# ctxnn/GenConViT

Hardware: AMD Instinct MI355X
Metric: frames/sec (224x224, ed+vae forward) (higher is better)
Workload: dtype f16

## Files before the change

genconvit_amd/_lib.py:

```python
from __future__ import annotations

import ctypes
import ctypes.util
import json
import os
import threading

_HERE = os.path.dirname(os.path.abspath(__file__))
LIB_PATH = os.environ.get("GCV_LIB_PATH") or os.path.join(_HERE, "lib", "libgenconvit_hip.so")

GCV_F32, GCV_BF16, GCV_F16 = 0, 1, 2
ACT_NONE, ACT_RELU, ACT_GELU, ACT_LEAKY = 0, 1, 2, 3
A_PLAIN, A_IM2COL3_POOL, A_IM2COL3_S2 = 0, 1, 2
EPI_BIAS_ACT, EPI_RESID, EPI_POOL4, EPI_CONVT, EPI_SPLITK = 0, 1, 2, 3, 4

c_void_p, c_int, c_int64, c_float, c_char_p, c_size_t = (ctypes.c_void_p, ctypes.c_int, ctypes.c_int64,
                                                         ctypes.c_float, ctypes.c_char_p, ctypes.c_size_t)


class TensorDesc(ctypes.Structure):
    _fields_ = [("name", c_char_p), ("data", c_void_p), ("numel", c_int64), ("on_device", c_int)]


class GemmArgs(ctypes.Structure):
# ... 30 lines not shown
    "gcv_comm_unique_id": (c_int, [c_void_p]),
    "gcv_comm_create": (c_int, [ctypes.POINTER(c_void_p), c_int, c_int, c_void_p, c_int]),
    "gcv_comm_destroy": (None, [c_void_p]),
    "gcv_allgather_logits": (c_int, [c_void_p, c_void_p, c_int, c_void_p, c_void_p]),
    "gcv_convnext_forward": (c_int, [c_void_p, c_int, c_void_p, c_int, c_int, c_void_p, c_void_p]),
    "gcv_swin_forward": (c_int, [c_void_p, c_void_p, c_int, c_void_p, c_void_p]),
    "gcv_vote": (c_int, [c_void_p, c_int, c_void_p, c_void_p]),
    "gcv_preprocess": (c_int, [c_int, c_void_p, c_void_p, c_int, c_int, c_int, c_void_p]),
    "gcv_face_crop_resize": (c_int, [c_void_p, c_int, c_int, c_int, c_void_p, c_int, c_void_p, c_int, c_void_p]),
    "gcv_cam_overlay": (c_int, [c_void_p, c_int, c_int, c_int, c_void_p, c_int, c_void_p, c_int, c_int, c_void_p, c_float,
                                c_int, c_void_p, c_void_p]),
    "gcv_vote_segments": (c_int, [c_void_p, c_int, c_int, c_void_p, c_int, c_void_p, c_void_p]),
    "gcv_tap_set": (c_int, [c_void_p, c_char_p, c_void_p, c_size_t]),
    "gcv_tap_clear": (c_int, [c_void_p]),
    "gcv_tap_written": (c_int, [c_void_p, c_char_p]),
    "gcv_profile_enable": (c_int, [c_void_p, c_int]),
    "gcv_profile_report": (c_char_p, [c_void_p]),
    "gcv_k_gemm": (c_int, [c_int, c_int, c_int, ctypes.POINTER(GemmArgs), c_void_p]),
    "gcv_k_stem_ln": (c_int, [c_int, c_void_p, c_int64, c_int64, c_int64, c_int64, c_void_p, c_void_p, c_void_p,
                              c_void_p, c_void_p, c_int, c_int, c_int, c_float, c_void_p]),
    "gcv_k_stem_ln_c": (c_int, [c_int, c_void_p, c_int64, c_int64, c_int64, c_int64, c_void_p, c_void_p, c_void_p,
                                c_void_p, c_void_p, c_int, c_int, c_int, c_int, c_float, c_void_p]),
    "gcv_k_dwconv7_ln": (c_int, [c_int, c_void_p, c_void_p, c_void_p, c_void_p, c_void_p, c_void_p, c_int, c_int,
                                 c_int, c_int, c_float, c_void_p]),
    "gcv_dw_plan": (c_int, [c_int, c_int, c_int, c_int, c_int, c_int, c_void_p]),
    "gcv_convnext_res_ok": (c_int, [c_int, c_int]),
    "gcv_k_ln_patchify": (c_int, [c_int, c_void_p, c_void_p, c_void_p, c_void_p, c_int, c_int, c_int, c_int, c_float,
                                  c_void_p]),
    "gcv_k_layernorm_rows": (c_int, [c_int, c_void_p, c_void_p, c_void_p, c_void_p, c_int64, c_int, c_float, c_void_p]),
    "gcv_k_pool_ln": (c_int, [c_int, c_void_p, c_void_p, c_void_p, c_void_p, c_int, c_int, c_int, c_float, c_void_p]),
    "gcv_k_conv3_first": (c_int, [c_int, c_void_p, c_int64, c_int64, c_int64, c_int64, c_void_p, c_void_p, c_void_p,
                                  c_int, c_int, c_int, c_int, c_int, c_void_p]),
    "gcv_k_convt2_small": (c_int, [c_int, c_void_p, c_void_p, c_void_p, c_void_p, c_int, c_int, c_int, c_int, c_void_p]),
    "gcv_k_reparam": (c_int, [c_int, c_void_p, c_int, c_void_p, c_void_p, c_void_p, c_void_p, c_int, c_int, c_void_p]),
    "gcv_k_head_tail": (c_int, [c_int, c_void_p, c_void_p, c_void_p, c_void_p, c_int, c_int, c_void_p]),
    "gcv_k_head_tail_splitk": (c_int, [c_int, c_void_p, c_int, c_void_p, c_int, c_void_p, c_void_p, c_void_p, c_int, c_int,
                                       c_void_p]),
    "gcv_k_resize_mse": (c_int, [c_int, c_void_p, c_void_p, c_void_p, c_void_p, c_void_p, c_int, c_void_p]),
    "gcv_k_swin_window_attn": (c_int, [c_int, c_void_p, c_void_p, c_void_p, c_int, c_int, c_int, c_int, c_int, c_int,
                                       c_void_p]),
    "gcv_k_patch_merge_ln": (c_int, [c_int, c_void_p, c_void_p, c_void_p, c_void_p, c_int, c_int, c_int, c_int, c_float,
                                     c_void_p]),
    "gcv_k_mean_tokens": (c_int, [c_int, c_void_p, c_void_p, c_int, c_int, c_int, c_void_p]),
    "gcv_k_fused_mlp": (c_int, [c_int, c_int, c_void_p, c_void_p, c_void_p, c_void_p, c_void_p, c_void_p, c_void_p,
                                c_void_p, c_int, c_void_p]),
    "gcv_k_fused_mlp_lnp": (c_int, [c_int, c_int, c_void_p, c_void_p, c_void_p, c_void_p, c_void_p, c_void_p, c_void_p,
                                    c_void_p, c_void_p, c_float, c_int, c_void_p, c_void_p, c_void_p, c_void_p, c_void_p,
                                    c_int, c_void_p]),
    "gcv_k_fused_mlp_timed": (c_int, [c_int, c_int, c_void_p, c_void_p, c_void_p, c_void_p, c_void_p, c_void_p,
                                      c_void_p, c_void_p, c_int, c_int, c_void_p, c_void_p]),
}

_lib = None
_lock = threading.Lock()


class GenConViTHipError(RuntimeError):
    pass


def _preload_hip_runtime():
    cands = []
    try:
        import torch
        cands.append(os.path.join(os.path.dirname(torch.__file__), "lib", "libamdhip64.so"))
    except Exception:
# ... 483 lines not shown
```

genconvit_amd/csrc/api.hip:

```cpp
#include "../../include/genconvit_hip.h"

#include <dlfcn.h>

#include <cstdio>
#include <cstdlib>
#include <cstring>
#include <map>
#include <mutex>
#include <set>
#include <sstream>
#include <vector>

#include "cnx_mlp.h"
#include "gemm.h"
#include "kernels.h"
#include "net.h"

namespace gcv {
static thread_local std::string g_err;
void set_error(const std::string& msg) { g_err = msg; }
const char* get_error() { return g_err.c_str(); }

int ensure_dynamic_lds(const void* fn, int bytes) {
  static std::mutex mu;
  static std::map<std::pair<const void*, int>, int> done;
  int dev = 0;
  GCV_CHECK_HIP(hipGetDevice(&dev));
  std::lock_guard<std::mutex> lk(mu);
  auto it = done.find({fn, dev});
  if (it != done.end() && it->second >= bytes) return 0;
  GCV_CHECK_HIP(hipFuncSetAttribute(fn, hipFuncAttributeMaxDynamicSharedMemorySize, bytes));
  done[{fn, dev}] = bytes;
  return 0;
}

hipEvent_t Profiler::get_event() {
  if (next_event == pool.size()) {
    hipEvent_t e;
    if (hipEventCreate(&e) != hipSuccess) return nullptr;
    pool.push_back(e);
  }
  return pool[next_event++];
}
Profiler::~Profiler() {
  for (hipEvent_t e : pool) (void)hipEventDestroy(e);
}
// ... 574 lines not shown
    return rc;
  };
  DISPATCH_DT(dtype, put(dw_plan<T>(p, nimg, H, W, C, aligned != 0)));
}

int gcv_convnext_res_ok(int arch, int res) { return cnx_res_ok(arch, res) ? 1 : 0; }

int gcv_k_ln_patchify(int dtype, const void* x, const float* w, const float* b, void* out, int nimg, int H, int W,
                      int C, float eps, gcv_stream s) {
  DISPATCH_DT(dtype, launch_ln_patchify<T>((const T*)x, w, b, (T*)out, nimg, H, W, C, eps, (hipStream_t)s));
}

int gcv_k_layernorm_rows(int dtype, const void* x, const float* w, const float* b, void* out, int64_t rows, int C,
                         float eps, gcv_stream s) {
  DISPATCH_DT(dtype, launch_layernorm_rows<T>((const T*)x, w, b, (T*)out, rows, C, eps, (hipStream_t)s));
}

int gcv_k_pool_ln(int dtype, const void* x, const float* w, const float* b, void* out, int nimg, int HW, int C,
                  float eps, gcv_stream s) {
  DISPATCH_DT(dtype, launch_pool_ln<T>((const T*)x, w, b, (T*)out, nimg, HW, C, eps, (hipStream_t)s));
}

int gcv_k_conv3_first(int dtype, const void* x, int64_t sb, int64_t sc, int64_t sy, int64_t sx, const float* wp,
                      const float* bias, void* out, int nimg, int H, int W, int pool, int act, gcv_stream s) {
  DISPATCH_DT(dtype, launch_conv3_first<T>((const T*)x, sb, sc, sy, sx, wp, bias, (T*)out, nimg, H, W, pool != 0, act,
                                           (hipStream_t)s));
}

int gcv_k_convt2_small(int dtype, const void* x, const float* wp, const float* bias, void* out, int nimg, int H,
                       int W, int act, gcv_stream s) {
  DISPATCH_DT(dtype, launch_convt2_small<T>((const T*)x, wp, bias, (T*)out, nimg, H, W, act, (hipStream_t)s));
}

int gcv_k_reparam(int dtype, const float* partial, int splitk, const float* bias, const float* eps, float* mu_out,
                  void* z_nhwc, int B, int N, gcv_stream s) {
  DISPATCH_DT(dtype, launch_reparam<T>(partial, splitk, bias, eps, mu_out, (T*)z_nhwc, B, N, (hipStream_t)s));
}

int gcv_k_head_tail(int dtype, const void* h, const float* w, const float* bias, float* logits, int B, int K,
                    gcv_stream s) {
  DISPATCH_DT(dtype, launch_head_tail<T>((const T*)h, w, bias, logits, B, K, (hipStream_t)s));
}

int gcv_k_head_tail_splitk(int dtype, const float* partial, int splitk, const float* b1, int act, const float* w,
                           const float* bias, float* logits, int B, int K, gcv_stream s) {
  DISPATCH_DT(dtype, launch_head_tail_splitk<T>(partial, splitk, b1, act, w, bias, logits, B, K, (hipStream_t)s));
}

int gcv_k_resize_mse(int dtype, const void* xhat, const void* img, void* recon, float* msepart, float* mse, int B,
                     gcv_stream s) {
  DISPATCH_DT(dtype, launch_resize_mse<T>((const T*)xhat, (const T*)img, (T*)recon, msepart, mse, B, (hipStream_t)s));
}

int gcv_k_swin_window_attn(int dtype, const void* qkv, const float* rpb, void* out, int nimg, int H, int W, int C,
                           int nH, int shift, gcv_stream s) {
  DISPATCH_DT(dtype, launch_swin_window_attn<T>((const T*)qkv, rpb, (T*)out, nimg, H, W, C, nH, shift, (hipStream_t)s));
}

int gcv_k_patch_merge_ln(int dtype, const void* x, const float* w, const float* b, void* out, int nimg, int H, int W,
                         int C, float eps, gcv_stream s) {
  DISPATCH_DT(dtype, launch_patch_merge_ln<T>((const T*)x, w, b, (T*)out, nimg, H, W, C, eps, (hipStream_t)s));
}

int gcv_k_mean_tokens(int dtype, const void* x, void* out, int nimg, int L, int C, gcv_stream s) {
  DISPATCH_DT(dtype, launch_mean_tokens<T>((const T*)x, (T*)out, nimg, L, C, (hipStream_t)s));
}
// ... 51 lines not shown
```

genconvit_amd/csrc/net_impl.h:

```cpp
#pragma once
#include <algorithm>
#include <cmath>
#include <cstdlib>
#include <cstring>

#include "cam.h"
#include "cam_bwd.h"
#include "cnx_mlp.h"
#include "gemm.h"
#include "kernels.h"
#include "net.h"
#include "swin.h"

namespace gcv {

template <typename T> inline T host_cvt(float v);
template <> inline float host_cvt<float>(float v) { return v; }
template <> inline half_t host_cvt<half_t>(float v) { return (half_t)v; }
template <> inline bf16_t host_cvt<bf16_t>(float v) {
  uint32_t u;
  std::memcpy(&u, &v, 4);
  uint16_t h;
  if ((u & 0x7fffffffu) > 0x7f800000u) h = (uint16_t)((u >> 16) | 0x40);
  else h = (uint16_t)((u + 0x7fffu + ((u >> 16) & 1u)) >> 16);
  bf16_t r;
  std::memcpy(&r, &h, 2);
  return r;
}

struct WeightStore {
  std::vector<void*> ptrs;
  size_t bytes = 0;
  ~WeightStore() { clear(); }
  void clear() {
    for (void* p : ptrs) (void)hipFree(p);
    ptrs.clear();
    bytes = 0;
  }
  void* raw(size_t n) {
    void* p = nullptr;
    if (hipMalloc(&p, n ? n : 16) != hipSuccess) return nullptr;
// ... 803 lines not shown
                       Dw + (int64_t)tok0[p] * C3, B, side3[p], 1e-6f};
        GCV_TRY(run("explain2.dw_ln_bwd", 2.0 * 49 * B * hw3[p] * C3, (sizeof(T) + 8.0) * (double)B * hw3[p] * C3,
                    [&] { return launch_dw_ln_bwd<T>(da, C3, cur); }));
        GCV_TRY(run("explain2.dw_dgrad_res", 2.0 * 49 * B * hw3[p] * C3, 12.0 * (double)B * hw3[p] * C3, [&] {
          return launch_dw_dgrad_res(Dw + (int64_t)tok0[p] * C3, k.dw_w, G + (int64_t)tok0[p] * C3, B, side3[p], C3, cur);
        }));
      }
    }
    GCV_TRY(run("explain2.scale_rows", 2.0 * M * C3, (sizeof(T) + 4.0) * (double)M * C3,
                [&] { return launch_scale_rows<T>(G, nullptr, Gt, invA, (int)M, C3, cur); }));
    GCV_TRY(dgemm("explain2.dx_wdown", Gt, bw.bwd_downt, Dh, 4 * C2, C3));
    Cam2Args ca{};
    for (int p = 0; p < 2; ++p) {
      DownLnBwdArgs da{in3[p].s2, bw.down[2].ln_w, Dh + (int64_t)tok0[p] * 4 * C2, invA + tok0[p], dA2 + tok2[p] * C2, B,
                       side2[p], 1e-6f};
      GCV_TRY(run("explain2.down_ln_bwd", 10.0 * B * side2[p] * side2[p] * C2, (sizeof(T) + 8.0) * (double)B * side2[p] * side2[p] * C2,
                  [&] { return launch_down_ln_bwd<T>(da, C2, cur); }));
      ca.A[p] = in3[p].s2; ca.dA2[p] = dA2 + tok2[p] * C2; ca.side[p] = side2[p];
      ca.cam_off[p] = p ? side2[0] * side2[0] : 0;
    }
    ca.npass = 2; ca.cam_ld = ex.cam_ld; ca.up_pass = up_pass; ca.B = B; ca.cam = ex.cam; ca.cam224 = ex.cam224; ca.alpha = alpha;
    GCV_TRY(run("explain2.cam", 4.0 * M2 * C2, (sizeof(T) + 4.0) * (double)M2 * C2 + (ex.cam224 ? 4.0 * B * 224 * 224 : 0.0),
                [&] { return launch_cam2<T>(ca, C2, cur); }));
    if (!taps.empty()) GCV_TRY(tap_net((std::string(net) + ".explain.alpha2").c_str(), alpha, (size_t)2 * B * C2 * sizeof(float)));
    return 0;
  }

  int check_batch(int B) {
    GCV_REQUIRE(B >= 1, "batch must be >= 1");
    GCV_REQUIRE(B <= max_batch, "batch exceeds the max_batch this handle was created with");
    return 0;
  }

  int ed_forward(const void* xv, int B, float* logits, hipStream_t s) override { return ed_run(xv, B, logits, s, nullptr); }
  int ed_explain(const void* xv, int B, float* logits, const Explain& ex, hipStream_t s) override {
    return ed_run(xv, B, logits, s, &ex);
  }
  int ed_run(const void* xv, int B, float* logits, hipStream_t s, const Explain* ex) {
    if (!arena.dry) {
      GCV_REQUIRE(has_ed, "ED weights not loaded (gcv_load_ed)");
      GCV_TRY(check_batch(B));
      GCV_REQUIRE(xv && logits, "null input/output");
      GCV_REQUIRE(!ex || ex->cam, "null map output");
    }
    GCV_REQUIRE(!ex || ex->layer == 2 || ex->layer == 3, "explain layer must be 2 or 3");
    cur = s;
    const T* x = (const T*)xv;
    if (!taps.empty()) tap_reset("ed");
    const ArenaScope scope(arena);
    T* e1 = arena.get<T>((int64_t)B * 112 * 112 * 16);
    T* e2 = arena.get<T>((int64_t)B * 56 * 56 * 32);
    T* e3 = arena.get<T>((int64_t)B * 28 * 28 * 64);
    T* e4 = arena.get<T>((int64_t)B * 14 * 14 * 128);
    T* e5 = arena.get<T>((int64_t)B * 7 * 7 * 256);
    T* d1 = arena.get<T>((int64_t)B * 14 * 14 * 128);
    T* d2 = arena.get<T>((int64_t)B * 28 * 28 * 64);
    T* d3 = arena.get<T>((int64_t)B * 56 * 56 * 32);
    T* d4 = arena.get<T>((int64_t)B * 112 * 112 * 16);
    T* rec = arena.get<T>((int64_t)B * 224 * 224 * 3);
    T* feat = arena.get<T>((int64_t)B * 2000);
    T* bbpre = ex ? arena.get<T>((int64_t)B * 2000) : nullptr;
    if (!arena.dry && arena.overflow) { set_error("workspace arena too small"); return -6; }

    GCV_TRY(run("ed.enc1_conv3_relu_pool", 2.0 * B * 224 * 224 * 16 * 27,
                sizeof(T) * (double)B * (3 * 224 * 224 + 16 * 112 * 112), [&] {
      return launch_conv3_first<T>(x, 3 * 224 * 224, 224 * 224, 224, 1, ed.enc1_w, ed.enc1_b, e1, B, 224, 224, true,
                                   ACT_RELU, cur);
    }));
    {
      const T* in[4] = {e1, e2, e3, e4};
      T* out[4] = {e2, e3, e4, e5};
      const int Hs[4] = {112, 56, 28, 14};
      const int cl[4] = {4, 5, 6, 7};
      for (int l = 0; l < 4; ++l) {
        GemmArgs g{};
        g.A = in[l]; g.Wt = ed.enc_w[l]; g.C = out[l]; g.bias = ed.enc_b[l];
        g.M = B * Hs[l] * Hs[l]; g.N = 2 << cl[l]; g.K = 9 << cl[l]; g.ldc = g.N; g.act = ACT_RELU; g.splitk = 1;
        g.H = Hs[l]; g.W = Hs[l]; g.cin_log2 = cl[l];
        GCV_TRY(gemm("ed.enc_conv3_relu_pool", g, A_IM2COL3_POOL, EPI_POOL4));
      }
    }
    {
      const T* in[4] = {e5, d1, d2, d3};
      T* out[4] = {d1, d2, d3, d4};
      const int Hs[4] = {7, 14, 28, 56};
      const int col[4] = {7, 6, 5, 4};
      for (int l = 0; l < 4; ++l) {
        GemmArgs g{};
        g.A = in[l]; g.lda = 2 << col[l]; g.Wt = ed.dec_w[l]; g.C = out[l]; g.bias = ed.dec_b[l];
        g.M = B * Hs[l] * Hs[l]; g.N = 4 << col[l]; g.K = 2 << col[l]; g.act = ACT_RELU; g.splitk = 1;
        g.H = Hs[l]; g.W = Hs[l]; g.cout_log2 = col[l];
        GCV_TRY(gemm("ed.dec_convT_relu", g, A_PLAIN, EPI_CONVT));
      }
    }
    GCV_TRY(run("ed.dec5_convT_relu", 2.0 * B * 112 * 112 * 16 * 12,
                sizeof(T) * (double)B * (16 * 112 * 112 + 3 * 224 * 224),
                [&] { return launch_convt2_small<T>(d4, ed.dec5_w, ed.dec5_b, rec, B, 112, 112, ACT_RELU, cur); }));
    Seg<T> segs[2];
    segs[0] = Seg<T>{rec, (int64_t)224 * 224 * 3, 1, 224 * 3, 3, B, 224, 224, feat, 2000, ACT_GELU};
    segs[1] = Seg<T>{x, (int64_t)3 * 224 * 224, 224 * 224, 224, 1, B, 224, 224, feat + 1000, 2000, ACT_GELU};
    const T* s3[2] = {nullptr, nullptr};
    Stage3In<T> in3[2];
    const float* head_part = nullptr;
    if (ex)
      for (int q = 0; q < 2; ++q) {
        segs[q].pre = bbpre + 1000 * q; segs[q].s3 = &s3[q];
        if (ex->layer == 2) segs[q].in3 = &in3[q];
      }
    const TapPass tp{"ed", 2, 0, {B, B}, {224, 224}, {224, 224}};
    GCV_TRY(run_convnext(bb_ed, segs, 2, false, taps.empty() ? nullptr : &tp));
    GCV_TRY(run_head(ed.head, feat, B, ACT_GELU, logits, ex ? &head_part : nullptr));
    if (ex) {
      const int hwp[2] = {49, 49}, side[2] = {7, 7}, off[2] = {0, 49}, side2[2] = {14, 14};
      GCV_TRY(explain_tail(bb_ed, ed.head, ACT_GELU, B, head_part, bbpre, logits, s3, hwp, side, off, 1, *ex, in3, side2, "ed"));
    }
    if (!taps.empty()) {
      const T* et[5] = {e1, e2, e3, e4, e5};
      const int64_t ee[5] = {112 * 112 * 16, 56 * 56 * 32, 28 * 28 * 64, 14 * 14 * 128, 7 * 7 * 256};
      const T* dt[4] = {d1, d2, d3, d4};
      const int64_t de[4] = {14 * 14 * 128, 28 * 28 * 64, 56 * 56 * 32, 112 * 112 * 16};
      for (int l = 0; l < 5; ++l) GCV_TRY(tap_net(("ed.e" + std::to_string(l + 1)).c_str(), et[l], B * ee[l] * sizeof(T)));
      for (int l = 0; l < 4; ++l) GCV_TRY(tap_net(("ed.d" + std::to_string(l + 1)).c_str(), dt[l], B * de[l] * sizeof(T)));
      GCV_TRY(tap_net("ed.rec", rec, (size_t)B * 224 * 224 * 3 * sizeof(T)));
      GCV_TRY(tap_net("ed.feat", feat, (size_t)B * 2000 * sizeof(T)));
    }
    return 0;
  }

  int vae_forward(const void* xv, const float* eps, int B, float* logits, void* recon224, float* mse, float* kl,
                  hipStream_t s) override {
// ... 54 lines not shown
    GCV_TRY(run("vae.enc1_conv3s2_bn_leaky", 2.0 * B * 112 * 112 * 16 * 27,
                sizeof(T) * (double)B * (3 * 224 * 224 + 16 * 112 * 112), [&] {
      return launch_conv3_first<T>(x, 3 * 224 * 224, 224 * 224, 224, 1, vae.enc1_w, vae.enc1_b, v1, B, 224, 224,
                                   false, ACT_LEAKY, cur);
    }));
    {
      const T* in[3] = {v1, v2, v3};
      T* out[3] = {v2, v3, v4};
      const int Hs[3] = {112, 56, 28};
      const int cl[3] = {4, 5, 6};
      for (int l = 0; l < 3; ++l) {
        GemmArgs g{};
        g.A = in[l]; g.Wt = vae.enc_w[l]; g.C = out[l]; g.bias = vae.enc_b[l];
        g.M = B * (Hs[l] / 2) * (Hs[l] / 2); g.N = 2 << cl[l]; g.K = 9 << cl[l]; g.ldc = g.N; g.act = ACT_LEAKY;
        g.splitk = 1; g.H = Hs[l]; g.W = Hs[l]; g.cin_log2 = cl[l];
        GCV_TRY(gemm("vae.enc_conv3s2_bn_leaky", g, A_IM2COL3_S2, EPI_BIAS_ACT));
      }
    }
    {
      GemmArgs g{};
      g.A = v4; g.lda = 25088; g.Wt = vae.mu_w; g.partial = part; g.M = B; g.N = 12544; g.K = 25088;
      g.splitk = SPLITK; g.k_per_split = KPS; g.act = ACT_NONE;
      GCV_TRY(gemm("vae.mu_gemm_splitk", g, A_PLAIN, EPI_SPLITK));
      GCV_TRY(run("vae.reparam", 4.0 * B * 12544, 4.0 * (SPLITK + 2) * (double)B * 12544, [&] {
        return launch_reparam<T>(part, SPLITK, vae.mu_b, eps, mu, z, B, 12544, cur);
      }));
      if (kl) {
        g.Wt = vae.var_w;
        GCV_TRY(gemm("vae.var_gemm_splitk", g, A_PLAIN, EPI_SPLITK));
        GCV_TRY(run("vae.kl", 6.0 * B * 12544, 4.0 * (SPLITK + 1) * (double)B * 12544,
                    [&] { return launch_kl(part, SPLITK, vae.var_b, mu, rowsum, kl, B, 12544, cur); }));
      }
    }
    {
      const T* in[3] = {z, d1, d2};
      T* out[3] = {d1, d2, d3};
      const int Hs[3] = {7, 14, 28};
      const int cin[3] = {256, 64, 32};
      const int col[3] = {6, 5, 4};
      for (int l = 0; l < 3; ++l) {
        GemmArgs g{};
        g.A = in[l]; g.lda = cin[l]; g.Wt = vae.dec_w[l]; g.C = out[l]; g.bias = vae.dec_b[l];
        g.M = B * Hs[l] * Hs[l]; g.N = 4 << col[l]; g.K = cin[l]; g.act = ACT_LEAKY; g.splitk = 1;
        g.H = Hs[l]; g.W = Hs[l]; g.cout_log2 = col[l];
        GCV_TRY(gemm("vae.dec_convT_leaky", g, A_PLAIN, EPI_CONVT));
      }
    }
    GCV_TRY(run("vae.dec4_convT_leaky", 2.0 * B * 56 * 56 * 16 * 12,
                sizeof(T) * (double)B * (16 * 56 * 56 + 3 * 112 * 112),
                [&] { return launch_convt2_small<T>(d3, vae.dec4_w, vae.dec4_b, xhat, B, 56, 56, ACT_LEAKY, cur); }));
    if (after_chain && !arena.dry) GCV_TRY(after_chain());
    if (split) { GCV_TRY(run_convnext(bb_vae, &segs[1], 1, true, tapping ? &tp1 : nullptr)); }
    else { GCV_TRY(run_convnext(bb_vae, segs, 2, false, tapping ? &tp0 : nullptr)); }
    join.now();
    if (tapping) {
      const T* vt[4] = {v1, v2, v3, v4};
      const int64_t ve[4] = {112 * 112 * 16, 56 * 56 * 32, 28 * 28 * 64, 14 * 14 * 128};
      const T* dt[3] = {d1, d2, d3};
      const int64_t de[3] = {14 * 14 * 64, 28 * 28 * 32, 56 * 56 * 16};
      for (int l = 0; l < 4; ++l) GCV_TRY(tap_net(("vae.v" + std::to_string(l + 1)).c_str(), vt[l], B * ve[l] * sizeof(T)));
      GCV_TRY(tap_net("vae.mu", mu, (size_t)B * 12544 * sizeof(float)));
      GCV_TRY(tap_net("vae.z", z, (size_t)B * 12544 * sizeof(T)));
      for (int l = 0; l < 3; ++l) GCV_TRY(tap_net(("vae.d" + std::to_string(l + 1)).c_str(), dt[l], B * de[l] * sizeof(T)));
      GCV_TRY(tap_net("vae.xhat", xhat, (size_t)B * 112 * 112 * 3 * sizeof(T)));
      GCV_TRY(tap_net("vae.feat", feat, (size_t)B * 2000 * sizeof(T)));
    }
    GCV_TRY(run_head(vae.head, feat, B, ACT_RELU, logits, ex ? &head_part : nullptr));
    if (ex) {
      const int hwp[2] = {49, 9}, side[2] = {7, 3}, off[2] = {0, 49}, side2[2] = {14, 7};
      GCV_TRY(explain_tail(bb_vae, vae.head, ACT_RELU, B, head_part, bbpre, logits, s3, hwp, side, off, 0, *ex, in3, side2, "vae"));
    }
    if (recon224 || mse) {
      GCV_TRY(run("vae.resize_mse", 30.0 * B * 224 * 224, sizeof(T) * (double)B * (3 * 112 * 112 + 6 * 224 * 224), [&] {
        return launch_resize_mse<T>(xhat, x, (T*)recon224, msepart, mse, B, cur);
      }));
    }
    return 0;
  }

  int convnext_forward(int which, const void* xv, int B, int res, void* logits1000, hipStream_t s) override {
    GCV_REQUIRE(which == 0 ? has_ed : has_vae, "backbone weights not loaded");
    GCV_TRY(check_batch(B));
    GCV_REQUIRE(cnx_res_ok(arch, res), cnx_res_rule(arch));
// ... 43 lines not shown
```

include/genconvit_hip.h:

```cpp
#ifndef GENCONVIT_HIP_H
#define GENCONVIT_HIP_H

#include <stddef.h>
#include <stdint.h>

#ifdef __cplusplus
extern "C" {
#endif

#if defined(GCV_BUILD)
#pragma GCC visibility push(default)
#endif

typedef struct gcv_handle gcv_handle;
typedef void* gcv_stream;

enum { GCV_F32 = 0, GCV_BF16 = 1, GCV_F16 = 2 };
enum { GCV_CONVNEXT_TINY = 0, GCV_CONVNEXT_LARGE = 1 };
enum { GCV_LARGE_MAX_BATCH = 256 };
enum { GCV_ACT_NONE = 0, GCV_ACT_RELU = 1, GCV_ACT_GELU = 2, GCV_ACT_LEAKY = 3 };

typedef struct {
  const char* name;
  const void* data;
// ... 70 lines not shown
int gcv_tap_clear(gcv_handle* h);
int gcv_tap_written(gcv_handle* h, const char* name);

enum { GCV_A_PLAIN = 0, GCV_A_IM2COL3_POOL = 1, GCV_A_IM2COL3_S2 = 2 };
enum { GCV_EPI_BIAS_ACT = 0, GCV_EPI_RESID = 1, GCV_EPI_POOL4 = 2, GCV_EPI_CONVT = 3, GCV_EPI_SPLITK = 4 };

typedef struct {
  const void* A; const void* Wt; void* C;
  const float* bias; const float* gamma; const void* resid; float* partial;
  int M, N, K, lda, ldc, act, splitk, k_per_split, H, W, cin_log2, cout_log2;
} gcv_gemm_args;

int gcv_k_gemm(int dtype, int a_mode, int epi, const gcv_gemm_args* a, gcv_stream s);
int gcv_k_stem_ln(int dtype, const void* x, int64_t sb, int64_t sc, int64_t sy, int64_t sx, const float* wp,
                  const float* bias, const float* lnw, const float* lnb, void* out, int nimg, int Ho, int Wo,
                  float eps, gcv_stream s);
int gcv_k_stem_ln_c(int dtype, const void* x, int64_t sb, int64_t sc, int64_t sy, int64_t sx, const float* wp,
                    const float* bias, const float* lnw, const float* lnb, void* out, int nimg, int Ho, int Wo, int C,
                    float eps, gcv_stream s);
int gcv_k_dwconv7_ln(int dtype, const void* x, const float* wdw, const float* bdw, const float* lnw,
                     const float* lnb, void* y, int nimg, int H, int W, int C, float eps, gcv_stream s);
int gcv_dw_plan(int dtype, int nimg, int H, int W, int C, int aligned, int* out5);
int gcv_convnext_res_ok(int arch, int res);
int gcv_k_ln_patchify(int dtype, const void* x, const float* w, const float* b, void* out, int nimg, int H, int W,
                      int C, float eps, gcv_stream s);
int gcv_k_layernorm_rows(int dtype, const void* x, const float* w, const float* b, void* out, int64_t rows, int C,
                         float eps, gcv_stream s);
int gcv_k_pool_ln(int dtype, const void* x, const float* w, const float* b, void* out, int nimg, int HW, int C,
                  float eps, gcv_stream s);
int gcv_k_conv3_first(int dtype, const void* x, int64_t sb, int64_t sc, int64_t sy, int64_t sx, const float* wp,
                      const float* bias, void* out, int nimg, int H, int W, int pool, int act, gcv_stream s);
int gcv_k_convt2_small(int dtype, const void* x, const float* wp, const float* bias, void* out, int nimg, int H,
                       int W, int act, gcv_stream s);
int gcv_k_reparam(int dtype, const float* partial, int splitk, const float* bias, const float* eps, float* mu_out,
                  void* z_nhwc, int B, int N, gcv_stream s);
int gcv_k_head_tail(int dtype, const void* h, const float* w, const float* bias, float* logits, int B, int K,
                    gcv_stream s);
int gcv_k_head_tail_splitk(int dtype, const float* partial, int splitk, const float* b1, int act, const float* w,
                           const float* bias, float* logits, int B, int K, gcv_stream s);
int gcv_k_resize_mse(int dtype, const void* xhat, const void* img, void* recon, float* msepart, float* mse, int B,
                     gcv_stream s);

int gcv_k_swin_window_attn(int dtype, const void* qkv, const float* rpb, void* out, int nimg, int H, int W, int C,
                           int nH, int shift, gcv_stream s);
int gcv_k_patch_merge_ln(int dtype, const void* x, const float* w, const float* b, void* out, int nimg, int H, int W,
                         int C, float eps, gcv_stream s);
int gcv_k_mean_tokens(int dtype, const void* x, void* out, int nimg, int L, int C, gcv_stream s);

int gcv_k_fused_mlp(int dtype, int C, const void* x, const void* w1, const float* b1, const float* w2_f32,
                    const float* b2, const float* gamma, const void* resid, void* out, int M, gcv_stream s);
int gcv_k_fused_mlp_lnp(int dtype, int C, const void* x, const void* w1, const float* b1, const float* w2_f32,
                        const float* b2, const float* gamma, const void* resid, const float* ln_w, const float* ln_b,
                        float eps, int nseg, const int* tok0, const int* hw, const int* wd, const int* out0, void* out, int M,
                        gcv_stream s);
int gcv_k_fused_mlp_timed(int dtype, int C, const void* x, const void* w1, const float* b1, const float* w2_f32,
                          const float* b2, const float* gamma, const void* resid, void* out, int M, int iters,
                          float* ms3, gcv_stream s);

#if defined(GCV_BUILD)
#pragma GCC visibility pop
#endif

#ifdef __cplusplus
}
#endif
#endif
// ... 1 lines not shown
```

Measured before the change: 18970.

## Fuse transposed-conv decoder stack into a single register-resident MFMA kernel

Replaces the per-layer decoder (four or three stride-2 transposed-conv GEMMs plus the small final convT) with one kernel per network. Each 32-row block starts from a 7x7 latent pixel, keeps the intermediate activations in registers across the upsampling tree, and writes only the final RGB output. This removes the global-memory round trips for the large intermediate feature maps and several kernel launches. In exchange, registers per thread rise (which may lower occupancy) and the path only applies to 16-bit dtypes when no taps are active.

```diff
diff --git a/genconvit_amd/_lib.py b/genconvit_amd/_lib.py
--- a/genconvit_amd/_lib.py
+++ b/genconvit_amd/_lib.py
@@ -86,6 +86,8 @@
     "gcv_k_conv3_first": (c_int, [c_int, c_void_p, c_int64, c_int64, c_int64, c_int64, c_void_p, c_void_p, c_void_p,
                                   c_int, c_int, c_int, c_int, c_int, c_void_p]),
     "gcv_k_convt2_small": (c_int, [c_int, c_void_p, c_void_p, c_void_p, c_void_p, c_int, c_int, c_int, c_int, c_void_p]),
+    "gcv_k_decoder_chain": (c_int, [c_int, c_int, c_void_p, c_void_p, c_void_p, c_void_p, c_void_p, c_void_p, c_void_p,
+                                    c_void_p, c_void_p, c_void_p, c_void_p, c_void_p, c_int, c_void_p]),
     "gcv_k_reparam": (c_int, [c_int, c_void_p, c_int, c_void_p, c_void_p, c_void_p, c_void_p, c_int, c_int, c_void_p]),
     "gcv_k_head_tail": (c_int, [c_int, c_void_p, c_void_p, c_void_p, c_void_p, c_int, c_int, c_void_p]),
     "gcv_k_head_tail_splitk": (c_int, [c_int, c_void_p, c_int, c_void_p, c_int, c_void_p, c_void_p, c_void_p, c_int, c_int,
diff --git a/genconvit_amd/csrc/api.hip b/genconvit_amd/csrc/api.hip
--- a/genconvit_amd/csrc/api.hip
+++ b/genconvit_amd/csrc/api.hip
@@ -12,6 +12,7 @@
 #include <vector>
 
 #include "cnx_mlp.h"
+#include "decoder_chain.h"
 #include "gemm.h"
 #include "kernels.h"
 #include "net.h"
@@ -652,6 +653,16 @@
   DISPATCH_DT(dtype, launch_convt2_small<T>((const T*)x, wp, bias, (T*)out, nimg, H, W, act, (hipStream_t)s));
 }
 
+int gcv_k_decoder_chain(int dtype, int net, const void* x, const void* w1, const float* b1, const void* w2,
+                        const float* b2, const void* w3, const float* b3, const void* w4, const float* b4,
+                        const float* w_last, const float* b_last, void* out, int B, gcv_stream s) {
+  GCV_REQUIRE(dtype == GCV_F16 || dtype == GCV_BF16, "the decoder chain is built for 16-bit storage");
+  GCV_REQUIRE(B > 0, "decoder chain: B >= 1");
+  const DecoderChainArgs a{x, {w1, w2, w3, w4}, {b1, b2, b3, b4}, w_last, b_last, out, B * 49};
+  if (dtype == GCV_F16) return launch_decoder_chain<half_t>(net, a, (hipStream_t)s);
+  return launch_decoder_chain<bf16_t>(net, a, (hipStream_t)s);
+}
+
 int gcv_k_reparam(int dtype, const float* partial, int splitk, const float* bias, const float* eps, float* mu_out,
                   void* z_nhwc, int B, int N, gcv_stream s) {
   DISPATCH_DT(dtype, launch_reparam<T>(partial, splitk, bias, eps, mu_out, (T*)z_nhwc, B, N, (hipStream_t)s));
diff --git a/genconvit_amd/csrc/decoder_chain.h b/genconvit_amd/csrc/decoder_chain.h
--- /dev/null
+++ b/genconvit_amd/csrc/decoder_chain.h
@@ -0,0 +1,230 @@
+#pragma once
+#include "common.h"
+#include "gemm.h"
+
+namespace gcv {
+
+struct DecoderChainArgs {
+  const void* x;
+  const void* w[4];
+  const float* b[4];
+  const float* w_last;
+  const float* b_last;
+  void* out;
+  int M;
+};
+
+template <typename T> int launch_decoder_chain(int net, const DecoderChainArgs& a, hipStream_t s);
+
+#ifdef GCV_DECODER_CHAIN_KERNELS
+
+typedef uint32_t u32x2 __attribute__((ext_vector_type(2)));
+typedef uint32_t u32x3 __attribute__((ext_vector_type(3)));
+
+template <typename T> __device__ __forceinline__ uint32_t dc_pack2(float a, float b) {
+  typedef T t2 __attribute__((ext_vector_type(2)));
+  return __builtin_bit_cast(uint32_t, (t2){from_f<T>(a), from_f<T>(b)});
+}
+
+template <typename T> __device__ __forceinline__ u32x4 dc_wfrag(const T* __restrict__ wrow, int s, int h) {
+  const u32x2 lo = *reinterpret_cast<const u32x2*>(wrow + 16 * s + 4 * h);
+  const u32x2 hi = *reinterpret_cast<const u32x2*>(wrow + 16 * s + 8 + 4 * h);
+  return u32x4{lo[0], lo[1], hi[0], hi[1]};
+}
+
+template <typename T, int ACT>
+__device__ __forceinline__ void dc_epi(const f32x16& acc, const float* sb, u32x4& k0, u32x4& k1) {
+  uint32_t p[8];
+#pragma unroll
+  for (int q = 0; q < 4; ++q) {
+    const f32x4 bv = *reinterpret_cast<const f32x4*>(sb + 8 * q);
+    float v[4];
+#pragma unroll
+    for (int e = 0; e < 4; ++e) v[e] = act_fn<ACT>(acc[4 * q + e] + bv[e]);
+    p[2 * q] = dc_pack2<T>(v[0], v[1]);
+    p[2 * q + 1] = dc_pack2<T>(v[2], v[3]);
+  }
+  k0 = u32x4{p[0], p[1], p[2], p[3]};
+  k1 = u32x4{p[4], p[5], p[6], p[7]};
+}
+
+__device__ __forceinline__ void dc_zero(f32x16& a) {
+#pragma unroll
+  for (int r = 0; r < 16; ++r) a[r] = 0.0f;
+}
+
+template <typename T, int NL, int ACT>
+__global__ void __launch_bounds__(256) decoder_chain_kernel(const DecoderChainArgs a) {
+  static_assert(sizeof(T) == 2, "the decoder chain is built for 16-bit storage");
+  static_assert(NL == 5 || NL == 4, "ED (5 layers) or VAE (4 layers)");
+  constexpr int C1 = NL == 5 ? 128 : 64;
+  constexpr int NB1 = C1 / 32;
+  constexpr int S = 7 << NL;
+  constexpr int OFF2 = C1;
+  constexpr int OFF3 = NL == 5 ? C1 + 64 : C1;
+  constexpr int OFF4 = OFF3 + 32;
+  constexpr int NBIAS = OFF4 + 16;
+  __shared__ __attribute__((aligned(16))) float sB[NBIAS];
+  __shared__ __attribute__((aligned(16))) float sW5[16 * 12];
+  __shared__ __attribute__((aligned(16))) float sB5[4];
+
+  const int tid = threadIdx.x, lane = tid & 63, wave = tid >> 6;
+  const int lr = lane & 31, h = lane >> 5;
+  const T* __restrict__ w3 = (const T*)a.w[NL - 3];
+  const T* __restrict__ w4 = (const T*)a.w[NL - 2];
+
+  if (tid < C1) sB[tid] = a.b[0][tid];
+  if (NL == 5 && tid < 64) sB[OFF2 + tid] = a.b[1][tid];
+  if (tid < 32) sB[OFF3 + tid] = a.b[NL - 3][tid];
+  if (tid < 16) sB[OFF4 + tid] = a.b[NL - 2][tid];
+  if (tid < 192) sW5[tid] = a.w_last[tid];
+  if (tid < 4) sB5[tid] = tid < 3 ? a.b_last[tid] : 0.0f;
+
+  u32x4 w3f[4][4], w4f[2][2];
+#pragma unroll
+  for (int d = 0; d < 4; ++d)
+#pragma unroll
+    for (int s = 0; s < 4; ++s) w3f[d][s] = dc_wfrag<T>(w3 + (d * 32 + lr) * 64, s, h);
+#pragma unroll
+  for (int nb = 0; nb < 2; ++nb) {
+    const int n = (2 * nb + ((lr >> 2) & 1)) * 16 + 4 * (lr >> 3) + (lr & 3);
+#pragma unroll
+    for (int s = 0; s < 2; ++s) w4f[nb][s] = dc_wfrag<T>(w4 + n * 32, s, h);
+  }
+
+  const int m = blockIdx.x * 32 + lr;
+  const bool live = m < a.M;
+  const int mc = live ? m : a.M - 1;
+  const int img = mc / 49, pix = mc - img * 49;
+  const int y0 = pix / 7, x0 = pix - y0 * 7;
+  T* __restrict__ outp = (T*)a.out + (int64_t)img * S * S * 3;
+
+  u32x4 a1[2 * NB1];
+  {
+    const T* __restrict__ xr = (const T*)a.x + (int64_t)mc * 256 + 8 * h;
+    u32x4 xf[16];
+#pragma unroll
+    for (int t = 0; t < 16; ++t) xf[t] = *reinterpret_cast<const u32x4*>(xr + 16 * t);
+    const T* __restrict__ w1 = (const T*)a.w[0] + (int64_t)(wave * C1 + lr) * 256 + 8 * h;
+    __syncthreads();
+#pragma unroll
+    for (int nb = 0; nb < NB1; ++nb) {
+      f32x16 acc;
+      dc_zero(acc);
+#pragma unroll
+      for (int t = 0; t < 16; ++t) {
+        const u32x4 wf = *reinterpret_cast<const u32x4*>(w1 + nb * 32 * 256 + 16 * t);
+        Mfma<T>::run(wf, xf[t], acc);
+      }
+      dc_epi<T, ACT>(acc, sB + nb * 32 + 4 * h, a1[2 * nb], a1[2 * nb + 1]);
+      __builtin_amdgcn_sched_barrier(0);
+    }
+  }
+  const int Y1 = 2 * y0 + (wave >> 1), X1 = 2 * x0 + (wave & 1);
+
+  auto tail = [&](const u32x4 (&a3)[4], int Y, int X) {
+#pragma unroll
+    for (int d3 = 0; d3 < 4; ++d3) {
+      f32x16 acc3;
+      dc_zero(acc3);
+#pragma unroll
+      for (int s = 0; s < 4; ++s) Mfma<T>::run(w3f[d3][s], a3[s], acc3);
+      u32x4 a4[2];
+      dc_epi<T, ACT>(acc3, sB + OFF3 + 4 * h, a4[0], a4[1]);
+      f32x16 acc4[2];
+#pragma unroll
+      for (int nb = 0; nb < 2; ++nb) {
+        dc_zero(acc4[nb]);
+#pragma unroll
+        for (int s = 0; s < 2; ++s) Mfma<T>::run(w4f[nb][s], a4[s], acc4[nb]);
+      }
+      float v[2][16];
+#pragma unroll
+      for (int q = 0; q < 4; ++q) {
+        const f32x4 bv = *reinterpret_cast<const f32x4*>(sB + OFF4 + 4 * q);
+#pragma unroll
+        for (int nb = 0; nb < 2; ++nb)
+#pragma unroll
+          for (int e = 0; e < 4; ++e)
+            v[nb][4 * q + e] = to_f(from_f<T>(act_fn<ACT>(acc4[nb][4 * q + e] + bv[e])));
+      }
+      f32x2 o[2][6];
+      const f32x4 b5 = *reinterpret_cast<const f32x4*>(sB5);
+#pragma unroll
+      for (int nb = 0; nb < 2; ++nb)
+#pragma unroll
+        for (int j = 0; j < 6; ++j) o[nb][j] = f32x2{b5[(2 * j) % 3], b5[(2 * j + 1) % 3]};
+#pragma unroll
+      for (int ci = 0; ci < 16; ++ci) {
+        if (ci % 4 == 0) __builtin_amdgcn_sched_barrier(0);
+        const f32x4* wr = reinterpret_cast<const f32x4*>(sW5 + ci * 12);
+#pragma unroll
+        for (int g = 0; g < 3; ++g) {
+          const f32x4 w = wr[g];
+          const f32x2 wl = {w[0], w[1]}, wh = {w[2], w[3]};
+#pragma unroll
+          for (int nb = 0; nb < 2; ++nb) {
+            o[nb][2 * g] = __builtin_elementwise_fma(splat2(v[nb][ci]), wl, o[nb][2 * g]);
+            o[nb][2 * g + 1] = __builtin_elementwise_fma(splat2(v[nb][ci]), wh, o[nb][2 * g + 1]);
+          }
+        }
+      }
+      if (live) {
+        const int Y3 = 2 * Y + (d3 >> 1), X3 = 2 * X + (d3 & 1);
+#pragma unroll
+        for (int nb = 0; nb < 2; ++nb) {
+          const int Y5 = 2 * (2 * Y3 + nb), X5 = 2 * (2 * X3 + h);
+#pragma unroll
+          for (int dy = 0; dy < 2; ++dy) {
+            uint32_t pk[3];
+#pragma unroll
+            for (int j = 0; j < 3; ++j)
+              pk[j] = dc_pack2<T>(apply_act(o[nb][3 * dy + j][0], ACT), apply_act(o[nb][3 * dy + j][1], ACT));
+            *reinterpret_cast<u32x3*>(outp + ((Y5 + dy) * S + X5) * 3) = u32x3{pk[0], pk[1], pk[2]};
+          }
+        }
+      }
+    }
+  };
+
+  if constexpr (NL == 4) {
+    tail(a1, Y1, X1);
+  } else {
+    const T* __restrict__ w2 = (const T*)a.w[1];
+#pragma unroll 1
+    for (int d2 = 0; d2 < 4; ++d2) {
+      u32x4 a3[4];
+#pragma unroll
+      for (int nb = 0; nb < 2; ++nb) {
+        const T* __restrict__ wrow = w2 + (d2 * 64 + nb * 32 + lr) * 128;
+        f32x16 acc;
+        dc_zero(acc);
+#pragma unroll
+        for (int s = 0; s < 8; ++s) Mfma<T>::run(dc_wfrag<T>(wrow, s, h), a1[s], acc);
+        dc_epi<T, ACT>(acc, sB + OFF2 + nb * 32 + 4 * h, a3[2 * nb], a3[2 * nb + 1]);
+        __builtin_amdgcn_sched_barrier(0);
+      }
+      tail(a3, 2 * Y1 + (d2 >> 1), 2 * X1 + (d2 & 1));
+    }
+  }
+}
+
+template <typename T> int launch_decoder_chain(int net, const DecoderChainArgs& a, hipStream_t s) {
+  GCV_REQUIRE(net == 0 || net == 1, "decoder chain: net is 0 (ED) or 1 (VAE)");
+  const int nl = net == 0 ? 4 : 3;
+  GCV_REQUIRE(a.M > 0 && a.M % 49 == 0, "decoder chain: M = B * 49 rows");
+  GCV_REQUIRE(a.x && a.out && a.w_last && a.b_last, "decoder chain: null argument");
+  auto al = [](const void* p, unsigned n) { return (reinterpret_cast<uintptr_t>(p) & (n - 1)) == 0; };
+  GCV_REQUIRE(al(a.x, 16) && al(a.out, 4), "decoder chain: x must be 16-byte and out 4-byte aligned");
+  for (int l = 0; l < nl; ++l)
+    GCV_REQUIRE(a.w[l] && a.b[l] && al(a.w[l], 16), "decoder chain: a layer's weights (16-byte aligned) or bias missing");
+  const dim3 grid((unsigned)cdiv(a.M, 32));
+  if (net == 0) hipLaunchKernelGGL((decoder_chain_kernel<T, 5, ACT_RELU>), grid, dim3(256), 0, s, a);
+  else hipLaunchKernelGGL((decoder_chain_kernel<T, 4, ACT_LEAKY>), grid, dim3(256), 0, s, a);
+  GCV_CHECK_HIP(hipGetLastError());
+  return 0;
+}
+
+#endif
+
+}
diff --git a/genconvit_amd/csrc/decoder_chain_bf16.hip b/genconvit_amd/csrc/decoder_chain_bf16.hip
--- /dev/null
+++ b/genconvit_amd/csrc/decoder_chain_bf16.hip
@@ -0,0 +1,5 @@
+#define GCV_DECODER_CHAIN_KERNELS
+#include "decoder_chain.h"
+namespace gcv {
+template int launch_decoder_chain<bf16_t>(int, const DecoderChainArgs&, hipStream_t);
+}
diff --git a/genconvit_amd/csrc/decoder_chain_f16.hip b/genconvit_amd/csrc/decoder_chain_f16.hip
--- /dev/null
+++ b/genconvit_amd/csrc/decoder_chain_f16.hip
@@ -0,0 +1,5 @@
+#define GCV_DECODER_CHAIN_KERNELS
+#include "decoder_chain.h"
+namespace gcv {
+template int launch_decoder_chain<half_t>(int, const DecoderChainArgs&, hipStream_t);
+}
diff --git a/genconvit_amd/csrc/net_impl.h b/genconvit_amd/csrc/net_impl.h
--- a/genconvit_amd/csrc/net_impl.h
+++ b/genconvit_amd/csrc/net_impl.h
@@ -7,6 +7,7 @@
 #include "cam.h"
 #include "cam_bwd.h"
 #include "cnx_mlp.h"
+#include "decoder_chain.h"
 #include "gemm.h"
 #include "kernels.h"
 #include "net.h"
@@ -876,6 +877,8 @@
     return 0;
   }
 
+  bool decoder_chain_ok() const { return sizeof(T) == 2 && taps.empty(); }
+
   int ed_forward(const void* xv, int B, float* logits, hipStream_t s) override { return ed_run(xv, B, logits, s, nullptr); }
   int ed_explain(const void* xv, int B, float* logits, const Explain& ex, hipStream_t s) override {
     return ed_run(xv, B, logits, s, &ex);
@@ -924,22 +927,31 @@
         GCV_TRY(gemm("ed.enc_conv3_relu_pool", g, A_IM2COL3_POOL, EPI_POOL4));
       }
     }
-    {
-      const T* in[4] = {e5, d1, d2, d3};
-      T* out[4] = {d1, d2, d3, d4};
-      const int Hs[4] = {7, 14, 28, 56};
-      const int col[4] = {7, 6, 5, 4};
-      for (int l = 0; l < 4; ++l) {
-        GemmArgs g{};
-        g.A = in[l]; g.lda = 2 << col[l]; g.Wt = ed.dec_w[l]; g.C = out[l]; g.bias = ed.dec_b[l];
-        g.M = B * Hs[l] * Hs[l]; g.N = 4 << col[l]; g.K = 2 << col[l]; g.act = ACT_RELU; g.splitk = 1;
-        g.H = Hs[l]; g.W = Hs[l]; g.cout_log2 = col[l];
-        GCV_TRY(gemm("ed.dec_convT_relu", g, A_PLAIN, EPI_CONVT));
-      }
-    }
-    GCV_TRY(run("ed.dec5_convT_relu", 2.0 * B * 112 * 112 * 16 * 12,
-                sizeof(T) * (double)B * (16 * 112 * 112 + 3 * 224 * 224),
-                [&] { return launch_convt2_small<T>(d4, ed.dec5_w, ed.dec5_b, rec, B, 112, 112, ACT_RELU, cur); }));
+    if (decoder_chain_ok()) {
+      if constexpr (sizeof(T) == 2) {
+        const DecoderChainArgs a{e5, {ed.dec_w[0], ed.dec_w[1], ed.dec_w[2], ed.dec_w[3]},
+                                 {ed.dec_b[0], ed.dec_b[1], ed.dec_b[2], ed.dec_b[3]}, ed.dec5_w, ed.dec5_b, rec, B * 49};
+        GCV_TRY(run("ed.dec_chain", 2.0 * B * 49 * (256.0 * 512 + 4 * 128 * 256 + 16 * 64 * 128 + 64 * 32 * 64 + 256 * 16 * 12),
+                    sizeof(T) * (double)B * (256 * 49 + 3 * 224 * 224), [&] { return launch_decoder_chain<T>(0, a, cur); }));
+      }
+    } else {
+      {
+        const T* in[4] = {e5, d1, d2, d3};
+        T* out[4] = {d1, d2, d3, d4};
+        const int Hs[4] = {7, 14, 28, 56};
+        const int col[4] = {7, 6, 5, 4};
+        for (int l = 0; l < 4; ++l) {
+          GemmArgs g{};
+          g.A = in[l]; g.lda = 2 << col[l]; g.Wt = ed.dec_w[l]; g.C = out[l]; g.bias = ed.dec_b[l];
+          g.M = B * Hs[l] * Hs[l]; g.N = 4 << col[l]; g.K = 2 << col[l]; g.act = ACT_RELU; g.splitk = 1;
+          g.H = Hs[l]; g.W = Hs[l]; g.cout_log2 = col[l];
+          GCV_TRY(gemm("ed.dec_convT_relu", g, A_PLAIN, EPI_CONVT));
+        }
+      }
+      GCV_TRY(run("ed.dec5_convT_relu", 2.0 * B * 112 * 112 * 16 * 12,
+                  sizeof(T) * (double)B * (16 * 112 * 112 + 3 * 224 * 224),
+                  [&] { return launch_convt2_small<T>(d4, ed.dec5_w, ed.dec5_b, rec, B, 112, 112, ACT_RELU, cur); }));
+    }
     Seg<T> segs[2];
     segs[0] = Seg<T>{rec, (int64_t)224 * 224 * 3, 1, 224 * 3, 3, B, 224, 224, feat, 2000, ACT_GELU};
     segs[1] = Seg<T>{x, (int64_t)3 * 224 * 224, 224 * 224, 224, 1, B, 224, 224, feat + 1000, 2000, ACT_GELU};
@@ -1060,23 +1072,32 @@
                     [&] { return launch_kl(part, SPLITK, vae.var_b, mu, rowsum, kl, B, 12544, cur); }));
       }
     }
-    {
-      const T* in[3] = {z, d1, d2};
-      T* out[3] = {d1, d2, d3};
-      const int Hs[3] = {7, 14, 28};
-      const int cin[3] = {256, 64, 32};
-      const int col[3] = {6, 5, 4};
-      for (int l = 0; l < 3; ++l) {
-        GemmArgs g{};
-        g.A = in[l]; g.lda = cin[l]; g.Wt = vae.dec_w[l]; g.C = out[l]; g.bias = vae.dec_b[l];
-        g.M = B * Hs[l] * Hs[l]; g.N = 4 << col[l]; g.K = cin[l]; g.act = ACT_LEAKY; g.splitk = 1;
-        g.H = Hs[l]; g.W = Hs[l]; g.cout_log2 = col[l];
-        GCV_TRY(gemm("vae.dec_convT_leaky", g, A_PLAIN, EPI_CONVT));
-      }
-    }
-    GCV_TRY(run("vae.dec4_convT_leaky", 2.0 * B * 56 * 56 * 16 * 12,
-                sizeof(T) * (double)B * (16 * 56 * 56 + 3 * 112 * 112),
-                [&] { return launch_convt2_small<T>(d3, vae.dec4_w, vae.dec4_b, xhat, B, 56, 56, ACT_LEAKY, cur); }));
+    if (decoder_chain_ok()) {
+      if constexpr (sizeof(T) == 2) {
+        const DecoderChainArgs a{z, {vae.dec_w[0], vae.dec_w[1], vae.dec_w[2], nullptr},
+                                 {vae.dec_b[0], vae.dec_b[1], vae.dec_b[2], nullptr}, vae.dec4_w, vae.dec4_b, xhat, B * 49};
+        GCV_TRY(run("vae.dec_chain", 2.0 * B * 49 * (256.0 * 256 + 4 * 64 * 128 + 16 * 32 * 64 + 64 * 16 * 12),
+                    sizeof(T) * (double)B * (256 * 49 + 3 * 112 * 112), [&] { return launch_decoder_chain<T>(1, a, cur); }));
+      }
+    } else {
+      {
+        const T* in[3] = {z, d1, d2};
+        T* out[3] = {d1, d2, d3};
+        const int Hs[3] = {7, 14, 28};
+        const int cin[3] = {256, 64, 32};
+        const int col[3] = {6, 5, 4};
+        for (int l = 0; l < 3; ++l) {
+          GemmArgs g{};
+          g.A = in[l]; g.lda = cin[l]; g.Wt = vae.dec_w[l]; g.C = out[l]; g.bias = vae.dec_b[l];
+          g.M = B * Hs[l] * Hs[l]; g.N = 4 << col[l]; g.K = cin[l]; g.act = ACT_LEAKY; g.splitk = 1;
+          g.H = Hs[l]; g.W = Hs[l]; g.cout_log2 = col[l];
+          GCV_TRY(gemm("vae.dec_convT_leaky", g, A_PLAIN, EPI_CONVT));
+        }
+      }
+      GCV_TRY(run("vae.dec4_convT_leaky", 2.0 * B * 56 * 56 * 16 * 12,
+                  sizeof(T) * (double)B * (16 * 56 * 56 + 3 * 112 * 112),
+                  [&] { return launch_convt2_small<T>(d3, vae.dec4_w, vae.dec4_b, xhat, B, 56, 56, ACT_LEAKY, cur); }));
+    }
     if (after_chain && !arena.dry) GCV_TRY(after_chain());
     if (split) { GCV_TRY(run_convnext(bb_vae, &segs[1], 1, true, tapping ? &tp1 : nullptr)); }
     else { GCV_TRY(run_convnext(bb_vae, segs, 2, false, tapping ? &tp0 : nullptr)); }
diff --git a/include/genconvit_hip.h b/include/genconvit_hip.h
--- a/include/genconvit_hip.h
+++ b/include/genconvit_hip.h
@@ -126,6 +126,9 @@
                       const float* bias, void* out, int nimg, int H, int W, int pool, int act, gcv_stream s);
 int gcv_k_convt2_small(int dtype, const void* x, const float* wp, const float* bias, void* out, int nimg, int H,
                        int W, int act, gcv_stream s);
+int gcv_k_decoder_chain(int dtype, int net, const void* x, const void* w1, const float* b1, const void* w2,
+                        const float* b2, const void* w3, const float* b3, const void* w4, const float* b4,
+                        const float* w_last, const float* b_last, void* out, int B, gcv_stream s);
 int gcv_k_reparam(int dtype, const float* partial, int splitk, const float* bias, const float* eps, float* mu_out,
                   void* z_nhwc, int B, int N, gcv_stream s);
 int gcv_k_head_tail(int dtype, const void* h, const float* w, const float* bias, float* logits, int B, int K,
diff --git a/profiles/decoder_chain_ab.py b/profiles/decoder_chain_ab.py
--- /dev/null
+++ b/profiles/decoder_chain_ab.py
@@ -0,0 +1,93 @@
+from __future__ import annotations
+
+import argparse
+import json
+import os
+import subprocess
+import sys
+
+ROOT = os.path.dirname(os.path.dirname(os.path.abspath(__file__)))
+CONFIGS = (("genconvit", 128, "f16"), ("vae", 32, "bf16"))
+
+
+def io_bytes(net, batch):
+    ed = 2 * batch * (49 * 256 + 224 * 224 * 3)
+    vae = 2 * batch * (49 * 256 + 112 * 112 * 3)
+    return {"ed": ed, "vae": vae, "genconvit": ed + vae}[net]
+
+
+def child(steps, warmup):
+    import torch
+    sys.path.insert(0, ROOT)
+    import bench
+    from genconvit_amd import synth
+    from genconvit_amd.model.genconvit import GenConViT
+    torch.set_grad_enabled(False)
+    device = torch.device("cuda", 0)
+    for net, batch, dt in CONFIGS:
+        dtype = bench.DT[dt]
+        model, _ = bench.build_models(net, dtype, batch, device)
+        x = synth.make_frames(batch, name="bench_frames_r0").to(device).to(dtype)
+        eps = synth.make_eps(batch, name="bench_eps_r0").to(device)
+        for _ in range(warmup):
+            model(x, eps=eps)
+        torch.cuda.synchronize()
+        handles = [m._handle for m in (getattr(model, "model_ed", None), getattr(model, "model_vae", None)) if m is not None]
+        for h in handles:
+            h.profile_enable(True)
+        GenConViT.concurrent = False
+        agg = {}
+        for ps in range(steps + 1):
+            model(x, eps=eps)
+            torch.cuda.synchronize()
+            for h in handles:
+                recs = h.profile_report()
+                if ps == 0:
+                    continue
+                for r in recs:
+                    g = agg.setdefault(r["tag"], {"launches": 0, "ms": 0.0})
+                    g["launches"] += r["launches"]
+                    g["ms"] += r["ms"]
+        for h in handles:
+            h.profile_enable(False)
+        dec = {t: v for t, v in agg.items() if ".dec" in t}
+        dec_ms = sum(v["ms"] for v in dec.values()) / steps
+        out = {"net": net, "batch": batch, "dtype": dt, "profiled_steps": steps,
+               "decoder_tags_ms_per_step": {t: round(v["ms"] / steps, 4) for t, v in sorted(dec.items())},
+               "decoder_launches_per_step": sum(v["launches"] for v in dec.values()) // steps,
+               "decoder_ms_per_step": round(dec_ms, 4),
+               "decoder_io_GBps": round(io_bytes(net, batch) / (dec_ms * 1e-3) / 1e9, 1),
+               "all_kernels_ms_per_step": round(sum(v["ms"] for v in agg.values()) / steps, 4)}
+        print("RESULT " + json.dumps(out), flush=True)
+        del model, handles, x, eps
+        torch.cuda.empty_cache()
+
+
+def main():
+    ap = argparse.ArgumentParser()
+    ap.add_argument("--lib", action="append", default=[], metavar="LABEL=PATH", help="a build of libgenconvit_hip.so (twice)")
+    ap.add_argument("--pairs", type=int, default=3)
+    ap.add_argument("--steps", type=int, default=10, help="profiled steps per measurement")
+    ap.add_argument("--warmup", type=int, default=3)
+    ap.add_argument("--child", action="store_true")
+    a = ap.parse_args()
+    if a.child:
+        return child(a.steps, a.warmup)
+    libs = [s.split("=", 1) for s in a.lib]
+    if len(libs) != 2:
+        ap.error("give two builds: --lib LABEL=PATH --lib LABEL=PATH")
+    for pair in range(a.pairs):
+        for label, path in libs:
+            env = dict(os.environ, GCV_LIB_PATH=os.path.abspath(path))
+            p = subprocess.run([sys.executable, os.path.abspath(__file__), "--child", "--steps", str(a.steps), "--warmup",
+                                str(a.warmup)], env=env, capture_output=True, text=True, timeout=600)
+            if p.returncode != 0:
+                sys.stderr.write(p.stderr[-4000:])
+                raise SystemExit(f"pair {pair} build {label}: the measurement exited with status {p.returncode}; stopping")
+            for line in p.stdout.splitlines():
+                if line.startswith("RESULT "):
+                    print(json.dumps(dict({"pair": pair, "build": label}, **json.loads(line[7:]))), flush=True)
+
+
+if __name__ == "__main__":
+    main()
```

Result: no change. 19070, median of 6 (+0.5%).
